# qcraftai/gedepth

Hardware: AMD Instinct MI355X
Metric: training img/s (whole node), KITTI-shaped 352x1120 synthetic batches (higher is better)
Workload: dtype bf16; 1 GPU; depthformer_swint_v: DepthFormer-SwinT + GEDepth-Vanilla, 352x1120, 8 img/GPU, full train step; global_batch=8, parallelism=dp1, allreduce_dtype=fp32, layout=nhwc, window_attention=bf16 mfma, params=53516992, hip_graph=off

## Files before the change

gedepth_amd/csrc/msda.h:

```cpp
#pragma once
#include <limits.h>
#include "common.h"

#define MSDA_MAX_L 8
struct MsdaLevels { int H[MSDA_MAX_L]; int W[MSDA_MAX_L]; int start[MSDA_MAX_L]; };

template <typename T> struct Lanes;
template <> struct Lanes<float> { static constexpr int CPL = 4; };
template <> struct Lanes<bf16_t> { static constexpr int CPL = 8; };

#define MSDA_XCDS 8
__device__ __forceinline__ long msda_xcd_block(unsigned bid, unsigned nblk) {
  return (long)(bid % MSDA_XCDS) * (nblk / MSDA_XCDS) + bid / MSDA_XCDS;
}
static inline unsigned msda_grid(long n_items, int per_block) {
  return (ge_blocks(n_items, per_block, INT_MAX - MSDA_XCDS) + MSDA_XCDS - 1) / MSDA_XCDS * MSDA_XCDS;
}

typedef ge_u32x4 lw_raw_t;
template <typename T> struct RowDot;
template <> struct RowDot<float> {
  static __device__ __forceinline__ float dot(const lw_raw_t& a, const lw_raw_t& b) {
    float s = 0.f;
#pragma unroll
    for (int i = 0; i < 4; ++i) s += __uint_as_float(a[i]) * __uint_as_float(b[i]);
    return s;
  }
};
template <> struct RowDot<bf16_t> {
  static __device__ __forceinline__ float dot(const lw_raw_t& a, const lw_raw_t& b) {
    const unsigned int a0 = a.x, a1 = a.y, a2 = a.z, a3 = a.w, b0 = b.x, b1 = b.y, b2 = b.z, b3 = b.w;
    float s = 0.f;
    s = __builtin_amdgcn_fdot2_f32_bf16(__builtin_bit_cast(ge_bf16x2, a0), __builtin_bit_cast(ge_bf16x2, b0), s, false);
    s = __builtin_amdgcn_fdot2_f32_bf16(__builtin_bit_cast(ge_bf16x2, a1), __builtin_bit_cast(ge_bf16x2, b1), s, false);
    s = __builtin_amdgcn_fdot2_f32_bf16(__builtin_bit_cast(ge_bf16x2, a2), __builtin_bit_cast(ge_bf16x2, b2), s, false);
    s = __builtin_amdgcn_fdot2_f32_bf16(__builtin_bit_cast(ge_bf16x2, a3), __builtin_bit_cast(ge_bf16x2, b3), s, false);
    return s;
  }
};

__device__ __forceinline__ int mul24(int a, int b) { return __mul24(a, b); }

static inline int msda_levels(const int* spatial_hw, int L, int Nv, MsdaLevels& lv) {
  if (L < 1 || L > MSDA_MAX_L) return GE_ERR_UNSUPPORTED;
  long start = 0;
  for (int l = 0; l < L; ++l) {
    lv.H[l] = spatial_hw[2 * l]; lv.W[l] = spatial_hw[2 * l + 1]; lv.start[l] = (int)start;
    if (lv.H[l] <= 0 || lv.W[l] <= 0) return GE_ERR_BAD_ARG;
    if ((long)lv.H[l] * lv.W[l] >= (1L << 23)) return GE_ERR_UNSUPPORTED;
    start += (long)lv.H[l] * lv.W[l];
  }
  return start == Nv ? GE_OK : GE_ERR_BAD_ARG;
}

#define MSDA_TW 8
#define MSDA_TH 4
#define MSDA_TILE 32
#define MSDA_CHUNK 4096
typedef float f32x32_t __attribute__((ext_vector_type(32)));
typedef float f32x2_t __attribute__((ext_vector_type(2)));
struct MsdaBins { int first_tile[MSDA_MAX_L + 1]; int ntx[MSDA_MAX_L]; };

struct MsdaWs {
  int* cnt; int* seg_hist; int* chunk_first; long* offset; int* ctrl; int4* entries;
  int* order;
};

int msda_drain_mfma_launch(const MsdaLevels& lv, const MsdaBins& bins, const MsdaWs& ws, const void* gout, float* d_value, int nbins,
                           int Nv, int Nq, int nH, int L, bool tr, hipStream_t s, bool rec8 = false);

int msda_win_supported(int B, int Nq, int nH, int L, int P, int Nv);
int msda_fwd_win_launch(const void* value, const MsdaLevels& lv, const int* query_hw, int n_qseg, const float* loc, const float* attw,
                        void* out, int B, int Nv, int Nq, int nH, int L, int P, int dtype, bool pre, hipStream_t s);
struct MwRaw {
  const void* off; long off_ld; const void* logit; long logit_ld;
  const float* ref; long ref_sb, ref_sq, ref_sl;
  float* loc_out; float* attw_out;
};
int msda_fwd_win_raw_launch(const void* value, const MsdaLevels& lv, const int* query_hw, int n_qseg, const MwRaw& rw, void* out, int B,
                            int Nv, int Nq, int nH, int L, int P, int dtype, hipStream_t s);
int msda_bwd_lw_win_launch(const void* value, const MsdaLevels& lv, const int* query_hw, int n_qseg, const float* loc,
                           const float* attw, const void* gout, float* d_loc, float* d_attw, int B, int Nv, int Nq, int nH, int L,
                           int P, int dtype, bool pre, hipStream_t s);
```

gedepth_amd/csrc/msda.hip:

```cpp
#include <algorithm>
#include <cstdlib>
#include "common.h"
#include "msda.h"
#include <string.h>
#include <mutex>
#include <vector>

__device__ __forceinline__ long msda_group(long v, int Nq, int nH, bool hm) {
  if (!hm) return v;
  const long bh = v / Nq;
  const long q = v - bh * Nq;
  const long b = bh / nH;
  return (b * Nq + q) * nH + (bh - b * nH);
}

template <typename T, bool HM>
__global__ void __launch_bounds__(256) msda_fwd_k(const T* __restrict__ value, MsdaLevels lv, const float* __restrict__ loc,
                                                  const float* __restrict__ attw, T* __restrict__ out,
                                                  long n_groups, int Nv, int Nq, int nH, int L, int P) {
  constexpr int CPL = Lanes<T>::CPL, G = 64 / CPL;
  const int c0 = (threadIdx.x % G) * CPL;
  const int nh64 = nH * 64;
  const long grp0 = msda_xcd_block(blockIdx.x, gridDim.x) * (blockDim.x / G) + (threadIdx.x / G);
  const long gstride = (long)gridDim.x * (blockDim.x / G);
// ... 495 lines not shown
            const float lg = bf2f(lgr[t]);
            const float e = __expf(lg - msda_half_max(lg));
            wgt = e * (1.f / msda_half_sum(e));
          }
          slot[s][0] = slot[s][1] = slot[s][2] = slot[s][3] = -1;
          key[s] = 0; packed[s] = 0;
          if (live && level_on && y > -1.f && x > -1.f && y < fH && x < fW) {
            const float xf = floorf(x), yf = floorf(y);
            const int x0 = (int)xf, y0 = (int)yf;
            const float ax = x - xf, ay = y - yf;
            const bool xa = x0 >= 0, xb = x0 + 1 < Wl, ya = y0 >= 0, yb = y0 + 1 < Hl;
            const int txa = x0 >> 3, txb = (x0 + 1) >> 3, tya = y0 >> 2, tyb = (y0 + 1) >> 2;
            const int tx = xa ? txa : txb, ty = ya ? tya : tyb;
            const bool two_x = xa && xb && txb != txa, two_y = ya && yb && tyb != tya;
            int* h0 = hist + lb0 + mul24(ty, ntx) + tx;
            const int lx1 = x0 - tx * MSDA_TW + 1, ly1 = y0 - ty * MSDA_TH + 1;
            key[s] = ((q_lo + (j >> 5)) << 7) | (ly1 << 4) | lx1;
            packed[s] = (uint32_t)f2bf(wgt) | ((uint32_t)min((int)(ax * 256.f), 255) << 16) | ((uint32_t)min((int)(ay * 256.f), 255) << 24);
            slot[s][0] = atomicAdd(h0, 1);
            if (two_x) slot[s][1] = atomicAdd(h0 + 1, 1);
            if (two_y) {
              slot[s][2] = atomicAdd(h0 + ntx, 1);
              if (two_x) slot[s][3] = atomicAdd(h0 + ntx + 1, 1);
            }
          }
        }
        if (FILL) {
          int2* rec = (int2*)ws.entries;
#pragma unroll
          for (int s = 0; s < S; ++s) {
            if (slot[s][0] >= 0) rec[slot[s][0]] = make_int2(key[s], (int)packed[s]);
            if (slot[s][1] >= 0) rec[slot[s][1]] = make_int2(key[s] & ~15, (int)packed[s]);
            if (slot[s][2] >= 0) rec[slot[s][2]] = make_int2(key[s] & ~0x70, (int)packed[s]);
            if (slot[s][3] >= 0) rec[slot[s][3]] = make_int2(key[s] & ~0x7f, (int)packed[s]);
          }
        }
      }
    }
    __syncthreads();
    if (!FILL) {
      for (int i = threadIdx.x; i < ntiles; i += 1024) {
        const int c = hist[i];
        gh[i] = c;
        if (c) atomicAdd(&ws.cnt[bh * ntiles + i], c);
      }
      __syncthreads();
    }
  }
}

__global__ void __launch_bounds__(256) msda_segscan_k(MsdaWs ws, int ntiles, int R, int nbins) {
  const int i = blockIdx.x * blockDim.x + threadIdx.x;
  if (i >= nbins) return;
  const int bh = i / ntiles, tile = i - bh * ntiles;
  int run = (int)ws.offset[i];
  int* p = ws.seg_hist + (long)bh * R * ntiles + tile;
  for (int r = 0; r < R; ++r) { const int c = p[(long)r * ntiles]; p[(long)r * ntiles] = run; run += c; }
}

__device__ __forceinline__ void msda_wave_scan(long& vo, int& vk, int lane) {
#pragma unroll
  for (int d = 1; d < 64; d <<= 1) {
    const long o = __shfl_up(vo, d, 64);
    const int k = __shfl_up(vk, d, 64);
    if (lane >= d) { vo += o; vk += k; }
  }
}
__global__ void __launch_bounds__(1024) msda_scan_k(MsdaWs ws, int nbins) {
  __shared__ long w_off[16];
  __shared__ int w_chk[16];
  const int lane = threadIdx.x & 63, wv = threadIdx.x >> 6;
  const int seg = ((nbins + 15) / 16 + 511) / 512 * 512;
  const int lo = wv * seg, hi = min(nbins, lo + seg);
  auto load8 = [&](int i0, int* c) {
    if (i0 + 8 <= hi) {
      const int4 a = *(const int4*)(ws.cnt + i0), b = *(const int4*)(ws.cnt + i0 + 4);
      c[0] = a.x; c[1] = a.y; c[2] = a.z; c[3] = a.w; c[4] = b.x; c[5] = b.y; c[6] = b.z; c[7] = b.w;
    } else {
#pragma unroll
      for (int e = 0; e < 8; ++e) c[e] = i0 + e < hi ? ws.cnt[i0 + e] : 0;
    }
  };
  long to = 0; int tk = 0;
  for (int base = lo; base < hi; base += 512) {
    int c[8];
    load8(base + lane * 8, c);
#pragma unroll
    for (int e = 0; e < 8; ++e) { to += c[e]; tk += (c[e] + MSDA_CHUNK - 1) / MSDA_CHUNK; }
  }
#pragma unroll
  for (int d = 32; d; d >>= 1) { to += __shfl_xor(to, d, 64); tk += __shfl_xor(tk, d, 64); }
  if (lane == 0) { w_off[wv] = to; w_chk[wv] = tk; }
  __syncthreads();
  long run_o = 0; int run_k = 0;
  for (int w = 0; w < wv; ++w) { run_o += w_off[w]; run_k += w_chk[w]; }
  for (int base = lo; base < hi; base += 512) {
    const int i0 = base + lane * 8;
    int c[8], kc[8];
    load8(i0, c);
    long vo = 0; int vk = 0;
#pragma unroll
    for (int e = 0; e < 8; ++e) { kc[e] = (c[e] + MSDA_CHUNK - 1) / MSDA_CHUNK; vo += c[e]; vk += kc[e]; }
    long so = vo; int sk = vk;
    msda_wave_scan(so, sk, lane);
    long o = run_o + so - vo; int k = run_k + sk - vk;
#pragma unroll
// ... 33 lines not shown
      int r = 0;
      for (int c = 0; c < nch; ++c) {
        const long slot = off0 + (long)c * MSDA_CHUNK;
        while (r + 1 < R && seg[(long)(r + 1) * ntiles + tile] <= slot) ++r;
        const int k = atomicAdd(&s_cnt[r], 1);
        if (pass) ws.order[first + s_base[r] + k] = c0 + c;
      }
    }
    __syncthreads();
    if (pass == 0) {
      if (threadIdx.x == 0) { int run = 0; for (int i = 0; i < R; ++i) { s_base[i] = run; run += s_cnt[i]; s_cnt[i] = 0; } }
      __syncthreads();
    }
  }
}

#define MSDA_SUB 512
#define MSDA_NCLS 45
template <typename T>
__global__ void __launch_bounds__(256) msda_drain_k(MsdaLevels lv, MsdaBins bins, MsdaWs ws, const T* __restrict__ gout,
                                                    float* __restrict__ d_value, int nbins, int Nv, int Nq, int nH, int L) {
  constexpr int CPLr = 16 / (int)sizeof(T);
  constexpr int LPR = 64 / CPLr;
  constexpr int RPI = 64 / LPR;
  constexpr int NR = 32 / RPI;
  __shared__ __attribute__((aligned(16))) T stage_all[4 * 32 * 64];
  __shared__ int s_key_all[4 * MSDA_SUB];
  __shared__ float s_w_all[4 * MSDA_SUB], s_ax_all[4 * MSDA_SUB], s_ay_all[4 * MSDA_SUB];
  __shared__ int s_start_all[4 * 64];
  const int lane = threadIdx.x & 63, wv = threadIdx.x >> 6;
  T* stage = stage_all + (size_t)wv * (32 * 64);
  int* s_key = s_key_all + wv * MSDA_SUB;
  float* s_w = s_w_all + wv * MSDA_SUB;
  float* s_ax = s_ax_all + wv * MSDA_SUB;
  float* s_ay = s_ay_all + wv * MSDA_SUB;
  int* s_start = s_start_all + wv * 64;
  const int gi = lane / LPR, subc = (lane % LPR) * CPLr;
  const int ntiles = bins.first_tile[L];
  const int total = ws.ctrl[0];
  const int part0 = blockIdx.x % MSDA_XCDS;
  int probe = 0;
  for (;;) {
    int item = -1;
    while (probe < MSDA_XCDS) {
      const int part = (part0 + probe) % MSDA_XCDS;
      const int p_lo = (int)((long)total * part / MSDA_XCDS), p_hi = (int)((long)total * (part + 1) / MSDA_XCDS);
      int k = 0;
      if (lane == 0) k = atomicAdd(&ws.ctrl[2 + part], 1);
      k = __builtin_amdgcn_readfirstlane(k);
      if (p_lo + k < p_hi) { item = p_lo + k; break; }
      ++probe;
    }
    if (item < 0) break;
    if (ws.order) item = ws.order[item];
    int lo = 0, hi = nbins;
    while (hi - lo > 1) { const int mid = (lo + hi) >> 1; if (ws.chunk_first[mid] <= item) lo = mid; else hi = mid; }
    const int bin = lo;
    const int nchunk = ws.chunk_first[bin + 1] - ws.chunk_first[bin];
    const int chunk = item - ws.chunk_first[bin];
    const int cnt = ws.cnt[bin];
    const int e_lo = chunk * MSDA_CHUNK, e_hi = min(cnt, e_lo + MSDA_CHUNK);
    const int4* ent = ws.entries + ws.offset[bin];
    const int bh = bin / ntiles, tile = bin - bh * ntiles;
    const int b = bh / nH, head = bh - b * nH;
    int l = 0;
    while (l + 1 < L && tile >= bins.first_tile[l + 1]) ++l;
    const int tl = tile - bins.first_tile[l];
    const int ty = tl / bins.ntx[l], tx = tl - ty * bins.ntx[l];
    const long rowbase = (long)b * Nq * nH + head;

    f32x32_t a0 = 0.f;
    for (int s_lo = e_lo; s_lo < e_hi; s_lo += MSDA_SUB) {
      const int n = min(MSDA_SUB, e_hi - s_lo);
      __builtin_amdgcn_wave_barrier();
      s_start[lane] = 0;
      __builtin_amdgcn_wave_barrier();
      int4 E[MSDA_SUB / 64];
      int rank[MSDA_SUB / 64];
#pragma unroll
      for (int i = 0; i < MSDA_SUB / 64; ++i) {
        const int idx = i * 64 + lane;
        E[i] = make_int4(0, 0, 0, 0);
        rank[i] = 0;
        if (idx < n) {
          E[i] = ent[s_lo + idx];
          rank[i] = atomicAdd(&s_start[((E[i].x >> 4) & 7) * 9 + (E[i].x & 15)], 1);
        }
      }
      __builtin_amdgcn_wave_barrier();
      {
        const int c = lane < MSDA_NCLS ? s_start[lane] : 0;
        int inc = c;
#pragma unroll
        for (int d = 1; d < 64; d <<= 1) { const int t = __shfl_up(inc, d, 64); if (lane >= d) inc += t; }
        __builtin_amdgcn_wave_barrier();
        s_start[lane] = lane < MSDA_NCLS ? inc - c : (lane == MSDA_NCLS ? n : 0x7fffffff);
      }
      __builtin_amdgcn_wave_barrier();
#pragma unroll
      for (int i = 0; i < MSDA_SUB / 64; ++i) {
        const int idx = i * 64 + lane;
        if (idx < n) {
          const int slot = s_start[((E[i].x >> 4) & 7) * 9 + (E[i].x & 15)] + rank[i];
          s_key[slot] = E[i].x;
          s_w[slot] = __int_as_float(E[i].y);
          s_ax[slot] = __int_as_float(E[i].z);
          s_ay[slot] = __int_as_float(E[i].w);
        }
      }
      const int nb = (n + 31) >> 5;
// ... 45 lines not shown
              accT = f32x2_t{carry ? accT.y : 0.f, 0.f};
              accB = f32x2_t{carry ? accB.y : 0.f, 0.f};
              ++cls;
              run_end = __builtin_amdgcn_readfirstlane(s_start[min(cls + 1, MSDA_NCLS + 1)]);
              rel = run_end - i0;
            } while (k == rel);
          }
          const f32x2_t kT = {nTx, nTy}, kB = {nBx, nBy};
          if (k + 1 < 32) {
            nTx = readlane_f(cT.x, k + 1); nTy = readlane_f(cT.y, k + 1); nBx = readlane_f(cB.x, k + 1); nBy = readlane_f(cB.y, k + 1);
          }
          const float g = gr[k];
          const f32x2_t g2 = {g, g};
          accT += kT * g2;
          accB += kB * g2;
        }
        if (blk + 1 < nb) { MSDA_PARK() }
      }
      {
        const int ly = cls / 9 - 1, lx = cls % 9 - 1;
        const bool in_cls = cls < MSDA_NCLS;
        MSDA_PUT(ly * MSDA_TW + lx, in_cls && ly >= 0 && lx >= 0, accT.x);
        MSDA_PUT((ly + 1) * MSDA_TW + lx, in_cls && ly < MSDA_TH - 1 && lx >= 0, accB.x);
        MSDA_PUT(ly * MSDA_TW + lx + 1, in_cls && ly >= 0 && lx < MSDA_TW - 1, accT.y);
        MSDA_PUT((ly + 1) * MSDA_TW + lx + 1, in_cls && ly < MSDA_TH - 1 && lx < MSDA_TW - 1, accB.y);
      }
#undef MSDA_GATHER
#undef MSDA_PARK
#undef MSDA_PUT
    }
    const int Wl = lv.W[l], Hl = lv.H[l];
    float* dst = d_value + (((long)b * Nv + lv.start[l]) * nH + head) * 64 + lane;
    const long pstride = (long)nH * 64;
#pragma unroll
    for (int e = 0; e < 32; ++e) {
      const int y = ty * MSDA_TH + e / MSDA_TW, x = tx * MSDA_TW + e % MSDA_TW;
      if (y < Hl && x < Wl) {
        float* p = dst + ((long)y * Wl + x) * pstride;
        if (nchunk == 1) *p = a0[e];
        else atomicAdd(p, a0[e]);
      }
    }
  }
}

static size_t msda_ws_layout(int nbins, long seg_hist_ints, long max_entries, char* base, MsdaWs* ws) {
  size_t off = 0;
  auto carve = [&](size_t bytes) { size_t o = off; off += (bytes + 255) / 256 * 256; return o; };
  const size_t o_cnt = carve((size_t)nbins * 4), o_chk = carve((size_t)(nbins + 1) * 4);
  const size_t o_off = carve((size_t)(nbins + 1) * 8), o_ctrl = carve(64), o_sh = carve((size_t)seg_hist_ints * 4);
  const size_t o_ord = carve((size_t)(nbins + max_entries / MSDA_CHUNK + 1) * 4);
  const size_t o_ent = carve((size_t)max_entries * 16);
  if (ws) {
    ws->order = (int*)(base + o_ord);
    ws->cnt = (int*)(base + o_cnt); ws->chunk_first = (int*)(base + o_chk); ws->offset = (long*)(base + o_off);
    ws->ctrl = (int*)(base + o_ctrl); ws->seg_hist = (int*)(base + o_sh); ws->entries = (int4*)(base + o_ent);
  }
  return off;
}
struct MsdaPlan { int ntiles, nloc, R, nbins; long max_entries; bool ok; };
#ifndef MSDA_HIST_WGS
#define MSDA_HIST_WGS 512
#endif
static MsdaPlan msda_plan(const MsdaBins& bins, int B, int Nq, int nH, int L, int P) {
  MsdaPlan pl;
  pl.ntiles = bins.first_tile[L];
  pl.nloc = nH * pl.ntiles;
  const long npts_b = (long)Nq * nH * L * P;
  long R = (MSDA_HIST_WGS + (long)B * nH - 1) / std::max(1L, (long)B * nH);
  R = std::max(1L, std::min(R, (long)std::max(1, Nq / 64)));
  pl.R = (int)R;
  pl.max_entries = (long)B * npts_b * 4;
  const long nbins = (long)B * pl.nloc;
  pl.nbins = (int)nbins;
  const size_t hist_bytes = (size_t)pl.ntiles * 4;
  pl.ok = nbins < (1L << 30) && Nq < (1 << 24) && pl.max_entries < (1L << 31) && hist_bytes <= 60 * 1024 && B <= 65535 &&
          ((long)Nq / R + 1) * L * P < (1L << 31) && (long)B * nH * R * pl.ntiles < (1L << 31) && R <= MSDA_MAX_R;
  return pl;
}
static int msda_bins(const MsdaLevels& lv, int L, MsdaBins& bins) {
  int n = 0;
  for (int l = 0; l < L; ++l) {
    bins.first_tile[l] = n;
    bins.ntx[l] = (lv.W[l] + MSDA_TW - 1) / MSDA_TW;
    n += bins.ntx[l] * ((lv.H[l] + MSDA_TH - 1) / MSDA_TH);
  }
  bins.first_tile[L] = n;
  return n;
}

static int g_msda_mode = 13 | 16 | 32;
extern "C" int ge_msda_mode(int mode) {
  const int old = g_msda_mode;
  if (mode >= 0) g_msda_mode = mode & 127;
  return old;
}

extern "C" int ge_msda_fwd(const void* value, const int* spatial_hw, const int* query_hw, int n_qseg, const float* loc,
                           const float* attw, void* out, int B, int Nv, int Nq, int nH, int L, int P, int dtype, void* stream) {
  if (!value || !spatial_hw || !loc || !attw || !out || B < 0 || Nv <= 0 || Nq < 0 || nH <= 0 || P <= 0) return GE_ERR_BAD_ARG;
  MsdaLevels lv;
  int e = msda_levels(spatial_hw, L, Nv, lv);
  if (e) return e;
  const long n_groups = (long)B * Nq * nH;
  if (n_groups == 0) return GE_OK;
  if (dtype != GE_F32 && dtype != GE_BF16) return GE_ERR_UNSUPPORTED;
  if ((g_msda_mode & 1) && query_hw && n_qseg > 0 && msda_win_supported(B, Nq, nH, L, P, Nv))
    return msda_fwd_win_launch(value, lv, query_hw, n_qseg, loc, attw, out, B, Nv, Nq, nH, L, P, dtype, (g_msda_mode & 4) != 0, ge_stream(stream));
  if ((n_groups + 15) / 16 > (1L << 30) || (long)Nv * nH * 64 >= (1L << 31)) return GE_ERR_UNSUPPORTED;
  const unsigned blocks = msda_grid(n_groups, dtype == GE_BF16 ? 32 : 16);
  const bool hm = (g_msda_mode & 8) != 0;
// ... 105 lines not shown
  const long seg_ints = (long)B * nH * pl.R * pl.ntiles;
  const bool binned = workspace && pl.ok && workspace_bytes >= msda_ws_layout(pl.nbins, seg_ints, pl.max_entries, nullptr, nullptr);
  if (!binned) {
    if (em || value_only) return GE_ERR_UNSUPPORTED;
    if (dtype == GE_F32) MSDA_BWD_P(float, true); else MSDA_BWD_P(bf16_t, true);
    GE_LAUNCH_CHECK();
    return GE_OK;
  }
#undef MSDA_BWD_P
#undef MSDA_BWD
  hipEvent_t evs[MSDA_NSTAGE + 1];
  hipEvent_t* ev = nullptr;
  { std::lock_guard<std::mutex> lk(g_msda_mu); if (g_msda_timing) ev = evs; }
  msda_mark(ev, 0, s);
  if (value_only) {
  } else if (em) {
    if (L != 4 || P != 8) return GE_ERR_UNSUPPORTED;
    const unsigned lblocks = msda_grid(n_groups, dtype == GE_BF16 ? 32 : 16);
    const bool hm = (g_msda_mode & 8) != 0;
    g_msda_lw_win_used = false;
#define MSDA_LWE(TT, HM_) msda_bwd_lw_k<TT, HM_, true><<<lblocks, 256, 0, s>>>((const TT*)value, lv, loc, attw, (const TT*)d_out, nullptr, nullptr, n_groups, Nv, Nq, nH, L, P, *em)
    if (dtype == GE_F32) { if (hm) MSDA_LWE(float, true); else MSDA_LWE(float, false); }
    else { if (hm) MSDA_LWE(bf16_t, true); else MSDA_LWE(bf16_t, false); }
#undef MSDA_LWE
  } else if ((g_msda_mode & 2) && query_hw && n_qseg > 0 && msda_win_supported(B, Nq, nH, L, P, Nv)) {
    e = msda_bwd_lw_win_launch(value, lv, query_hw, n_qseg, loc, attw, d_out, d_loc, d_attw, B, Nv, Nq, nH, L, P, dtype, (g_msda_mode & 4) != 0, s);
    if (e) return e;
    g_msda_lw_win_used = true;
  } else {
    const unsigned lblocks = msda_grid(n_groups, dtype == GE_BF16 ? 32 : 16);
    const bool hm = (g_msda_mode & 8) != 0;
    g_msda_lw_win_used = false;
#define MSDA_LW(TT, HM_) msda_bwd_lw_k<TT, HM_><<<lblocks, 256, 0, s>>>((const TT*)value, lv, loc, attw, (const TT*)d_out, d_loc, d_attw, n_groups, Nv, Nq, nH, L, P)
    if (dtype == GE_F32) { if (hm) MSDA_LW(float, true); else MSDA_LW(float, false); }
    else { if (hm) MSDA_LW(bf16_t, true); else MSDA_LW(bf16_t, false); }
#undef MSDA_LW
  }
  GE_LAUNCH_CHECK();
  msda_mark(ev, 1, s);
  if (!d_value) {
    if (ev) { std::lock_guard<std::mutex> lk(g_msda_mu); g_msda_pending.push_back(MsdaStageRec{0, ev[0], ev[1]}); }
    return GE_OK;
  }
  const int nbins = pl.nbins;
  MsdaWs ws;
  msda_ws_layout(nbins, seg_ints, pl.max_entries, (char*)workspace, &ws);
  hipError_t he = hipMemsetAsync(ws.cnt, 0, (size_t)nbins * 4, s);
  if (he != hipSuccess) return (int)he;
  const unsigned hgrid = (unsigned)std::min((long)MSDA_HIST_WGS, (long)B * nH * pl.R);
  const size_t hsmem = (size_t)pl.ntiles * 4;
  msda_hist_k<false><<<hgrid, 1024, hsmem, s>>>(lv, bins, loc, attw, ws, Nq, nH, L, P, pl.R, B);
  GE_LAUNCH_CHECK();
  msda_mark(ev, 2, s);
  msda_scan_k<<<1, 1024, 0, s>>>(ws, nbins);
  GE_LAUNCH_CHECK();
  msda_segscan_k<<<(unsigned)((nbins + 255) / 256), 256, 0, s>>>(ws, pl.ntiles, pl.R, nbins);
  GE_LAUNCH_CHECK();
  if (g_msda_mode & 64) {
    msda_order_k<<<(unsigned)(B * nH), 1024, 0, s>>>(ws, pl.ntiles, pl.R, 1);
    GE_LAUNCH_CHECK();
  } else ws.order = nullptr;
  msda_mark(ev, 3, s);
  msda_hist_k<true><<<hgrid, 1024, hsmem, s>>>(lv, bins, loc, attw, ws, Nq, nH, L, P, pl.R, B);
  GE_LAUNCH_CHECK();
  msda_mark(ev, 4, s);
  g_msda_drain_mfma_used = dtype == GE_BF16 && (g_msda_mode & 16);
  if (dtype == GE_F32)
    msda_drain_k<float><<<256 * 3, 256, 0, s>>>(lv, bins, ws, (const float*)d_out, d_value, nbins, Nv, Nq, nH, L);
  else if (g_msda_drain_mfma_used) {
    e = msda_drain_mfma_launch(lv, bins, ws, d_out, d_value, nbins, Nv, Nq, nH, L, (g_msda_mode & 32) != 0, s);
    if (e) return e;
  } else
    msda_drain_k<bf16_t><<<256 * 3, 256, 0, s>>>(lv, bins, ws, (const bf16_t*)d_out, d_value, nbins, Nv, Nq, nH, L);
  GE_LAUNCH_CHECK();
  msda_mark(ev, 5, s);
  if (ev) {
    std::lock_guard<std::mutex> lk(g_msda_mu);
    for (int i = 0; i < MSDA_NSTAGE; ++i) g_msda_pending.push_back(MsdaStageRec{i, ev[i], ev[i + 1]});
  }
  return GE_OK;
}

extern "C" int ge_msda_bwd(const void* value, const int* spatial_hw, const int* query_hw, int n_qseg, const float* loc,
                           const float* attw, const void* d_out, float* d_value, float* d_loc, float* d_attw, void* workspace,
                           size_t workspace_bytes, int B, int Nv, int Nq, int nH, int L, int P, int dtype, void* stream) {
  return msda_bwd_impl(value, spatial_hw, query_hw, n_qseg, loc, attw, d_out, d_value, d_loc, d_attw, workspace, workspace_bytes, B, Nv, Nq,
                       nH, L, P, dtype, stream, nullptr);
}

extern "C" int ge_msda_bwd_value(const void* value, const int* spatial_hw, const float* loc, const float* attw, const void* d_out,
                                 float* d_value, void* workspace, size_t workspace_bytes, int B, int Nv, int Nq, int nH, int L, int P,
                                 int dtype, void* stream) {
  return msda_bwd_impl(value, spatial_hw, nullptr, 0, loc, attw, d_out, d_value, nullptr, nullptr, workspace, workspace_bytes, B, Nv, Nq,
                       nH, L, P, dtype, stream, nullptr, true);
}

extern "C" int ge_msda_bwd_value_raw(const int* spatial_hw, const void* off_raw, long off_ld, const void* logit_raw, long logit_ld,
                                     const float* ref, long ref_sb, long ref_sq, long ref_sl, const void* d_out, float* d_value,
                                     void* workspace, size_t workspace_bytes, int B, int Nv, int Nq, int nH, int L, int P, int dtype,
                                     void* stream) {
  return ge_msda_bwd_value_raw_levels(spatial_hw, off_raw, off_ld, logit_raw, logit_ld, ref, ref_sb, ref_sq, ref_sl, d_out, d_value, workspace,
                                      workspace_bytes, 15, B, Nv, Nq, nH, L, P, dtype, stream);
}

extern "C" int ge_msda_bwd_value_raw_levels(const int* spatial_hw, const void* off_raw, long off_ld, const void* logit_raw, long logit_ld,
                                            const float* ref, long ref_sb, long ref_sq, long ref_sl, const void* d_out, float* d_value,
                                            void* workspace, size_t workspace_bytes, int level_mask, int B, int Nv, int Nq, int nH, int L,
                                            int P, int dtype, void* stream) {
  if (!spatial_hw || !off_raw || !logit_raw || !ref || !d_out || !d_value || !workspace || B < 0 || Nq < 0 || nH <= 0) return GE_ERR_BAD_ARG;
  if (dtype != GE_BF16 || L != 4 || P != 8) return GE_ERR_UNSUPPORTED;
  MsdaLevels lv;
  int e = msda_levels(spatial_hw, L, Nv, lv);
  if (e) return e;
  for (int l = 0; l < L; ++l) if (lv.W[l] > 8191 || lv.H[l] > 8191) return GE_ERR_UNSUPPORTED;
  if ((long)B * Nq * nH == 0) return GE_OK;
  MsdaBins bins;
  msda_bins(lv, L, bins);
  const MsdaPlan pl = msda_plan(bins, B, Nq, nH, L, P);
  const long seg_ints = (long)B * nH * pl.R * pl.ntiles;
  if (!pl.ok || workspace_bytes < msda_ws_layout(pl.nbins, seg_ints, pl.max_entries, nullptr, nullptr)) return GE_ERR_UNSUPPORTED;
  hipStream_t s = ge_stream(stream);
  MsdaRawIn in;
  in.off = (const bf16_t*)off_raw; in.off_ld = off_ld; in.logit = (const bf16_t*)logit_raw; in.logit_ld = logit_ld;
  in.ref = ref; in.ref_sb = ref_sb; in.ref_sq = ref_sq; in.ref_sl = ref_sl;
  for (int l = 0; l < 4; ++l) { in.fW[l] = (float)lv.W[l]; in.fH[l] = (float)lv.H[l]; in.rW[l] = 1.f / in.fW[l]; in.rH[l] = 1.f / in.fH[l]; }
  hipEvent_t evs[MSDA_NSTAGE + 1];
  hipEvent_t* ev = nullptr;
  { std::lock_guard<std::mutex> lk(g_msda_mu); if (g_msda_timing) ev = evs; }
  msda_mark(ev, 0, s);
  msda_mark(ev, 1, s);
  const int nbins = pl.nbins;
  MsdaWs ws;
  msda_ws_layout(nbins, seg_ints, pl.max_entries, (char*)workspace, &ws);
  hipError_t he = hipMemsetAsync(ws.cnt, 0, (size_t)nbins * 4, s);
  if (he != hipSuccess) return (int)he;
  const unsigned hgrid = (unsigned)std::min((long)MSDA_HIST_WGS, (long)B * nH * pl.R);
  const size_t hsmem = (size_t)pl.ntiles * 4;
  msda_hist_raw_k<false, MSDA_HIST_UC, 1><<<hgrid, 1024, hsmem, s>>>(lv, bins, in, ws, Nq, nH, pl.R, B, level_mask);
  GE_LAUNCH_CHECK();
  msda_mark(ev, 2, s);
  msda_scan_k<<<1, 1024, 0, s>>>(ws, nbins);
  GE_LAUNCH_CHECK();
  msda_segscan_k<<<(unsigned)((nbins + 255) / 256), 256, 0, s>>>(ws, pl.ntiles, pl.R, nbins);
  GE_LAUNCH_CHECK();
  if (g_msda_mode & 64) {
    msda_order_k<<<(unsigned)(B * nH), 1024, 0, s>>>(ws, pl.ntiles, pl.R, 1);
    GE_LAUNCH_CHECK();
  } else ws.order = nullptr;
  msda_mark(ev, 3, s);
  msda_hist_raw_k<true, MSDA_HIST_UF, MSDA_HIST_S><<<hgrid, 1024, hsmem, s>>>(lv, bins, in, ws, Nq, nH, pl.R, B, level_mask);
  GE_LAUNCH_CHECK();
  msda_mark(ev, 4, s);
  g_msda_drain_mfma_used = true;
  g_msda_lw_win_used = false;
  e = msda_drain_mfma_launch(lv, bins, ws, d_out, d_value, nbins, Nv, Nq, nH, L, true, s, true);
  if (e) return e;
  msda_mark(ev, 5, s);
  if (ev) {
    std::lock_guard<std::mutex> lk(g_msda_mu);
    for (int i = 0; i < MSDA_NSTAGE; ++i) g_msda_pending.push_back(MsdaStageRec{i, ev[i], ev[i + 1]});
  }
  return GE_OK;
}

template <typename T, int K>
__device__ __forceinline__ void ld_run(const T* p, float* v) {
  constexpr int VN = V8<T>::N;
  if constexpr (K % VN == 0) {
#pragma unroll
    for (int i = 0; i < K; i += VN) V8<T>::ld(p + i, v + i);
  } else {
#pragma unroll
    for (int i = 0; i < K; ++i) v[i] = Io<T>::ld(p + i);
  }
}
template <typename T, int K>
__device__ __forceinline__ void st_run(T* p, const float* v) {
  constexpr int VN = V8<T>::N;
  if constexpr (K % VN == 0) {
#pragma unroll
    for (int i = 0; i < K; i += VN) V8<T>::st(p + i, v + i);
  } else {
#pragma unroll
    for (int i = 0; i < K; ++i) Io<T>::st(p + i, v[i]);
  }
}

template <typename T, int P>
__global__ void __launch_bounds__(256) msda_prep_fwd_k(const T* __restrict__ off_raw, long off_ld, const T* __restrict__ logit_raw,
                                                       long logit_ld, const float* __restrict__ ref, long ref_sb, long ref_sq,
                                                       long ref_sl, MsdaLevels lv, float* __restrict__ loc, float* __restrict__ attw,
                                                       long total, int Nq, int nH) {
  for (long t = (long)blockIdx.x * 256 + threadIdx.x; t < total; t += (long)gridDim.x * 256) {
    const int l = (int)(t & 3);
    const long g = t >> 2;
    const int h = (int)(g % nH);
    const long row = g / nH;
    const long b = row / Nq, q = row - b * Nq;
    float off[2 * P], lg[P];
    ld_run<T, 2 * P>(off_raw + row * off_ld + ((long)h * 4 + l) * (2 * P), off);
    ld_run<T, P>(logit_raw + row * logit_ld + ((long)h * 4 + l) * P, lg);
// ... 205 lines not shown
```

gedepth_amd/csrc/msda_drain_mfma.hip:

```cpp
#include "msda.h"

#define MD_BLK 64
#define MD_HALF (MD_BLK * 32 + 32)
#define MD_STAGE (2 * MD_HALF)
#define MD_AIMG (MD_BLK * 32)

template <bool REC8> struct MdRec;
typedef int md_i32x4 __attribute__((ext_vector_type(4)));
typedef int md_i32x2 __attribute__((ext_vector_type(2)));
template <> struct MdRec<false> {
  typedef int4 T;
  static __device__ __forceinline__ T load(const T* p) { const md_i32x4 v = __builtin_nontemporal_load((const md_i32x4*)p); return make_int4(v.x, v.y, v.z, v.w); }
  static __device__ __forceinline__ T pad(int key) { return make_int4(key, 0, 0, 0); }
  static __device__ __forceinline__ int key(const T& e) { return e.x; }
  static __device__ __forceinline__ void coef(const T& e, float& w, float& ax, float& ay) { w = __int_as_float(e.y); ax = __int_as_float(e.z); ay = __int_as_float(e.w); }
};
template <> struct MdRec<true> {
  typedef int2 T;
  static __device__ __forceinline__ T load(const T* p) { const md_i32x2 v = __builtin_nontemporal_load((const md_i32x2*)p); return make_int2(v.x, v.y); }
  static __device__ __forceinline__ T pad(int key) { return make_int2(key, 0); }
  static __device__ __forceinline__ int key(const T& e) { return e.x; }
  static __device__ __forceinline__ void coef(const T& e, float& w, float& ax, float& ay) {
    w = __uint_as_float((uint32_t)e.y << 16);
    ax = ((float)(((uint32_t)e.y >> 16) & 255u) + 0.5f) * (1.f / 256.f);
    ay = ((float)((uint32_t)e.y >> 24) + 0.5f) * (1.f / 256.f);
  }
};

template <bool TR, bool REC8>
__global__ void __launch_bounds__(256) msda_drain_mfma_k(MsdaLevels lv, MsdaBins bins, MsdaWs ws, const bf16_t* __restrict__ gout,
                                                         float* __restrict__ d_value, int nbins, int Nv, int Nq, int nH, int L) {
  __shared__ __attribute__((aligned(16))) bf16_t stage_all[4 * MD_STAGE];
  __shared__ __attribute__((aligned(16))) bf16_t aimg_all[4 * MD_AIMG];
  const int lane = threadIdx.x & 63, wv = threadIdx.x >> 6;
  bf16_t* stage = stage_all + wv * MD_STAGE;
  bf16_t* aimg = aimg_all + wv * MD_AIMG;
  {
    const uint4 z = make_uint4(0, 0, 0, 0);
#pragma unroll
    for (int i = 0; i < MD_AIMG / (64 * 8); ++i) *(uint4*)(aimg + (i * 64 + lane) * 8) = z;
  }
  const int ntiles = bins.first_tile[L];
  const int total = ws.ctrl[0];
  const int part0 = blockIdx.x % MSDA_XCDS;
  const int sub8 = lane & 7, row8 = lane >> 3;
  const int park_off = (sub8 >> 2) * MD_HALF + (sub8 & 3) * 8;
  const int a_rec = ((lane >> 4) * 2 + ((lane >> 3) & 1)) * 256 + (lane & 7);
  const int tr_row = (lane >> 5) * 8 + ((lane & 15) >> 2), tr_col = ((lane >> 4) & 1) * 16 + (lane & 3) * 4;
  int probe = 0;
  for (;;) {
    int item = -1;
    while (probe < MSDA_XCDS) {
      const int part = (part0 + probe) % MSDA_XCDS;
      const int p_lo = (int)((long)total * part / MSDA_XCDS), p_hi = (int)((long)total * (part + 1) / MSDA_XCDS);
      int k = 0;
      if (lane == 0) k = atomicAdd(&ws.ctrl[2 + part], 1);
      k = __builtin_amdgcn_readfirstlane(k);
      if (p_lo + k < p_hi) { item = p_lo + k; break; }
      ++probe;
    }
    if (item < 0) break;
    if (ws.order) item = ws.order[item];
    int lo = 0, hi = nbins;
    while (hi - lo > 1) { const int mid = (lo + hi) >> 1; if (ws.chunk_first[mid] <= item) lo = mid; else hi = mid; }
    const int bin = lo;
    const int nchunk = ws.chunk_first[bin + 1] - ws.chunk_first[bin];
    const int chunk = item - ws.chunk_first[bin];
    const int cnt = ws.cnt[bin];
    const int e_lo = chunk * MSDA_CHUNK, e_hi = min(cnt, e_lo + MSDA_CHUNK);
    typedef typename MdRec<REC8>::T rec_t;
    const rec_t* ent = (const rec_t*)ws.entries + ws.offset[bin] + e_lo;
    const int n = e_hi - e_lo;
    const int bh = bin / ntiles, tile = bin - bh * ntiles;
    const int b = bh / nH, head = bh - b * nH;
    int l = 0;
    while (l + 1 < L && tile >= bins.first_tile[l + 1]) ++l;
    const int tl = tile - bins.first_tile[l];
    const int ty = tl / bins.ntx[l], tx = tl - ty * bins.ntx[l];
    const bf16_t* grow = gout + ((long)b * Nq * nH + head) * 64 + sub8 * 8;
    const int qpitch = nH * 64;

    ge_f32x16 acc0 = 0.f, acc1 = 0.f;
    const int nb = (n + MD_BLK - 1) / MD_BLK;
    ge_u32x4 R[8];
    rec_t E0, E1, E2;
    const rec_t padrec = MdRec<REC8>::pad(MdRec<REC8>::key(ent[0]));
#define MD_LOAD(DST, BLK) { DST = padrec; if ((BLK) * MD_BLK + lane < n) DST = MdRec<REC8>::load(ent + (BLK) * MD_BLK + lane); }
#define MD_GATHER(EE)                                                                          \
  _Pragma("unroll") for (int i = 0; i < 8; ++i) {                                              \
    const int q = __shfl(MdRec<REC8>::key(EE) >> 7, i * 8 + row8, 64);                                       \
    R[i] = *(const ge_u32x4*)(grow + (long)q * qpitch);                                         \
  }
#define MD_PARK()                                                                              \
  _Pragma("unroll") for (int i = 0; i < 8; ++i) *(ge_u32x4*)(stage + park_off + (i * 8 + row8) * 32) = R[i];
#define MD_COEF(EE, ZERO)                                                                      \
  {                                                                                            \
    const int lx = (MdRec<REC8>::key(EE) & 15) - 1, ly = ((MdRec<REC8>::key(EE) >> 4) & 7) - 1; \
    float w, ax, ay;                                                                            \
    MdRec<REC8>::coef(EE, w, ax, ay);                                                           \
    const bool xl = lx >= 0, xr = lx < MSDA_TW - 1, yt = ly >= 0, yb = ly < MSDA_TH - 1;        \
    const float wl = 1.f - ax, wt = w * (1.f - ay), wb = w * ay;                                \
    bf16_t* a00 = aimg + a_rec + (ly * MSDA_TW + lx) * 8;                                       \
    if (yt && xl) a00[0] = (ZERO) ? (bf16_t)0 : f2bf_hw(wt * wl);                                 \
    if (yt && xr) a00[8] = (ZERO) ? (bf16_t)0 : f2bf_hw(wt * ax);                                 \
    if (yb && xl) a00[MSDA_TW * 8] = (ZERO) ? (bf16_t)0 : f2bf_hw(wb * wl);                       \
    if (yb && xr) a00[MSDA_TW * 8 + 8] = (ZERO) ? (bf16_t)0 : f2bf_hw(wb * ax);                   \
  }
    MD_LOAD(E0, 0)
    MD_LOAD(E1, 1)
    MD_GATHER(E0)
    __builtin_amdgcn_wave_barrier();
    MD_COEF(E0, false)
    MD_PARK()
    __builtin_amdgcn_wave_barrier();
    for (int blk = 0; blk < nb; ++blk) {
      const bool more = blk + 1 < nb;
      if (more) { MD_GATHER(E1) }
      MD_LOAD(E2, blk + 2)
#pragma unroll
      for (int ks = 0; ks < 4; ++ks) {
        const ge_bf16x8 A = *(const ge_bf16x8*)(aimg + ((ks * 2 + (lane >> 5)) * 32 + (lane & 31)) * 8);
#pragma unroll
        for (int half = 0; half < 2; ++half) {
          ge_bf16x8 Bv;
          if (TR) {
            const bf16_t* p = stage + half * MD_HALF + (ks * 16 + tr_row) * 32 + tr_col;
            const ge_bf16x4 t0 = __builtin_amdgcn_ds_read_tr16_b64_v4bf16(GE_LDS(ge_bf16x4, p));
            const ge_bf16x4 t1 = __builtin_amdgcn_ds_read_tr16_b64_v4bf16(GE_LDS(ge_bf16x4, p + 4 * 32));
            Bv = __builtin_shufflevector(t0, t1, 0, 1, 2, 3, 4, 5, 6, 7);
          } else {
            const bf16_t* p = stage + half * MD_HALF + (ks * 16 + (lane >> 5) * 8) * 32 + (lane & 31);
            uint32_t wq[4];
#pragma unroll
            for (int e = 0; e < 4; ++e) wq[e] = (uint32_t)p[(2 * e) * 32] | ((uint32_t)p[(2 * e + 1) * 32] << 16);
            Bv = __builtin_bit_cast(ge_bf16x8, make_uint4(wq[0], wq[1], wq[2], wq[3]));
          }
          if (half == 0) acc0 = __builtin_amdgcn_mfma_f32_32x32x16_bf16(A, Bv, acc0, 0, 0, 0);
          else acc1 = __builtin_amdgcn_mfma_f32_32x32x16_bf16(A, Bv, acc1, 0, 0, 0);
        }
      }
      __builtin_amdgcn_wave_barrier();
      MD_COEF(E0, true)
      if (more) {
        MD_COEF(E1, false)
        MD_PARK()
      }
      __builtin_amdgcn_wave_barrier();
      E0 = E1; E1 = E2;
    }
#undef MD_LOAD
#undef MD_GATHER
#undef MD_PARK
#undef MD_COEF
    const int Wl = lv.W[l], Hl = lv.H[l];
    float* dst = d_value + (((long)b * Nv + lv.start[l]) * nH + head) * 64 + (lane & 31);
    const long pstride = (long)nH * 64;
#pragma unroll
    for (int r = 0; r < 16; ++r) {
      const int m = (r & 3) + 8 * (r >> 2) + 4 * (lane >> 5);
      const int y = ty * MSDA_TH + m / MSDA_TW, x = tx * MSDA_TW + m % MSDA_TW;
      if (y < Hl && x < Wl) {
        float* p = dst + ((long)y * Wl + x) * pstride;
        if (nchunk == 1) { p[0] = acc0[r]; p[32] = acc1[r]; }
        else { atomicAdd(p, acc0[r]); atomicAdd(p + 32, acc1[r]); }
      }
    }
  }
}

int msda_drain_mfma_launch(const MsdaLevels& lv, const MsdaBins& bins, const MsdaWs& ws, const void* gout, float* d_value, int nbins,
                           int Nv, int Nq, int nH, int L, bool tr, hipStream_t s, bool rec8) {
  if (rec8) msda_drain_mfma_k<true, true><<<256 * 3, 256, 0, s>>>(lv, bins, ws, (const bf16_t*)gout, d_value, nbins, Nv, Nq, nH, L);
  else if (tr) msda_drain_mfma_k<true, false><<<256 * 3, 256, 0, s>>>(lv, bins, ws, (const bf16_t*)gout, d_value, nbins, Nv, Nq, nH, L);
  else msda_drain_mfma_k<false, false><<<256 * 3, 256, 0, s>>>(lv, bins, ws, (const bf16_t*)gout, d_value, nbins, Nv, Nq, nH, L);
  GE_LAUNCH_CHECK();
  return GE_OK;
}
```

Measured before the change: 172.1 img/s.

## Deepen MSDA drain gather ring and precompute chunk-to-bin map

The MFMA drain kernel for the deformable-attention backward value gradient now keeps a ring of D gathered blocks and 2D entry records in flight, unrolling the block loop so that global gathers run further ahead of the MFMA work. It also sets an occupancy hint of three waves per SIMD, makes scalar values wave-uniform with readfirstlane, and clears coefficients by the previous key rather than through a separate zero pass. When ordering is off, the segscan kernel fills a chunk-to-bin table so the drain can skip its per-item binary search. The deeper ring raises register pressure, which the static_assert notes could spill.

```diff
diff --git a/gedepth_amd/csrc/msda.h b/gedepth_amd/csrc/msda.h
--- a/gedepth_amd/csrc/msda.h
+++ b/gedepth_amd/csrc/msda.h
@@ -56,7 +56,9 @@
 #define MSDA_TW 8
 #define MSDA_TH 4
 #define MSDA_TILE 32
+#ifndef MSDA_CHUNK
 #define MSDA_CHUNK 4096
+#endif
 typedef float f32x32_t __attribute__((ext_vector_type(32)));
 typedef float f32x2_t __attribute__((ext_vector_type(2)));
 struct MsdaBins { int first_tile[MSDA_MAX_L + 1]; int ntx[MSDA_MAX_L]; };
@@ -64,7 +66,16 @@
 struct MsdaWs {
   int* cnt; int* seg_hist; int* chunk_first; long* offset; int* ctrl; int4* entries;
   int* order;
+  int* chunk_bin;
 };
+
+__device__ __forceinline__ int msda_chunk_bin(const MsdaWs& ws, int& item, int nbins) {
+  if (ws.chunk_bin) return ws.chunk_bin[item];
+  item = ws.order[item];
+  int lo = 0, hi = nbins;
+  while (hi - lo > 1) { const int mid = (lo + hi) >> 1; if (ws.chunk_first[mid] <= item) lo = mid; else hi = mid; }
+  return lo;
+}
 
 int msda_drain_mfma_launch(const MsdaLevels& lv, const MsdaBins& bins, const MsdaWs& ws, const void* gout, float* d_value, int nbins,
                            int Nv, int Nq, int nH, int L, bool tr, hipStream_t s, bool rec8 = false);
diff --git a/gedepth_amd/csrc/msda.hip b/gedepth_amd/csrc/msda.hip
--- a/gedepth_amd/csrc/msda.hip
+++ b/gedepth_amd/csrc/msda.hip
@@ -571,6 +571,7 @@
 __global__ void __launch_bounds__(256) msda_segscan_k(MsdaWs ws, int ntiles, int R, int nbins) {
   const int i = blockIdx.x * blockDim.x + threadIdx.x;
   if (i >= nbins) return;
+  if (ws.chunk_bin) for (int ch = ws.chunk_first[i], end = ws.chunk_first[i + 1]; ch < end; ++ch) ws.chunk_bin[ch] = i;
   const int bh = i / ntiles, tile = i - bh * ntiles;
   int run = (int)ws.offset[i];
   int* p = ws.seg_hist + (long)bh * R * ntiles + tile;
@@ -710,10 +711,7 @@
       ++probe;
     }
     if (item < 0) break;
-    if (ws.order) item = ws.order[item];
-    int lo = 0, hi = nbins;
-    while (hi - lo > 1) { const int mid = (lo + hi) >> 1; if (ws.chunk_first[mid] <= item) lo = mid; else hi = mid; }
-    const int bin = lo;
+    const int bin = msda_chunk_bin(ws, item, nbins);
     const int nchunk = ws.chunk_first[bin + 1] - ws.chunk_first[bin];
     const int chunk = item - ws.chunk_first[bin];
     const int cnt = ws.cnt[bin];
@@ -865,11 +863,14 @@
   const size_t o_ord = carve((size_t)(nbins + max_entries / MSDA_CHUNK + 1) * 4);
   const size_t o_ent = carve((size_t)max_entries * 16);
   if (ws) {
-    ws->order = (int*)(base + o_ord);
+    ws->order = (int*)(base + o_ord); ws->chunk_bin = nullptr;
     ws->cnt = (int*)(base + o_cnt); ws->chunk_first = (int*)(base + o_chk); ws->offset = (long*)(base + o_off);
     ws->ctrl = (int*)(base + o_ctrl); ws->seg_hist = (int*)(base + o_sh); ws->entries = (int4*)(base + o_ent);
   }
   return off;
+}
+static void msda_ws_order(MsdaWs& ws, bool grouped) {
+  if (!grouped) { ws.chunk_bin = ws.order; ws.order = nullptr; }
 }
 struct MsdaPlan { int ntiles, nloc, R, nbins; long max_entries; bool ok; };
 #ifndef MSDA_HIST_WGS
@@ -1081,6 +1082,7 @@
   msda_hist_k<false><<<hgrid, 1024, hsmem, s>>>(lv, bins, loc, attw, ws, Nq, nH, L, P, pl.R, B);
   GE_LAUNCH_CHECK();
   msda_mark(ev, 2, s);
+  msda_ws_order(ws, (g_msda_mode & 64) != 0);
   msda_scan_k<<<1, 1024, 0, s>>>(ws, nbins);
   GE_LAUNCH_CHECK();
   msda_segscan_k<<<(unsigned)((nbins + 255) / 256), 256, 0, s>>>(ws, pl.ntiles, pl.R, nbins);
@@ -1088,7 +1090,7 @@
   if (g_msda_mode & 64) {
     msda_order_k<<<(unsigned)(B * nH), 1024, 0, s>>>(ws, pl.ntiles, pl.R, 1);
     GE_LAUNCH_CHECK();
-  } else ws.order = nullptr;
+  }
   msda_mark(ev, 3, s);
   msda_hist_k<true><<<hgrid, 1024, hsmem, s>>>(lv, bins, loc, attw, ws, Nq, nH, L, P, pl.R, B);
   GE_LAUNCH_CHECK();
@@ -1168,6 +1170,7 @@
   msda_hist_raw_k<false, MSDA_HIST_UC, 1><<<hgrid, 1024, hsmem, s>>>(lv, bins, in, ws, Nq, nH, pl.R, B, level_mask);
   GE_LAUNCH_CHECK();
   msda_mark(ev, 2, s);
+  msda_ws_order(ws, (g_msda_mode & 64) != 0);
   msda_scan_k<<<1, 1024, 0, s>>>(ws, nbins);
   GE_LAUNCH_CHECK();
   msda_segscan_k<<<(unsigned)((nbins + 255) / 256), 256, 0, s>>>(ws, pl.ntiles, pl.R, nbins);
@@ -1175,7 +1178,7 @@
   if (g_msda_mode & 64) {
     msda_order_k<<<(unsigned)(B * nH), 1024, 0, s>>>(ws, pl.ntiles, pl.R, 1);
     GE_LAUNCH_CHECK();
-  } else ws.order = nullptr;
+  }
   msda_mark(ev, 3, s);
   msda_hist_raw_k<true, MSDA_HIST_UF, MSDA_HIST_S><<<hgrid, 1024, hsmem, s>>>(lv, bins, in, ws, Nq, nH, pl.R, B, level_mask);
   GE_LAUNCH_CHECK();
diff --git a/gedepth_amd/csrc/msda_drain_mfma.hip b/gedepth_amd/csrc/msda_drain_mfma.hip
--- a/gedepth_amd/csrc/msda_drain_mfma.hip
+++ b/gedepth_amd/csrc/msda_drain_mfma.hip
@@ -27,9 +27,21 @@
   }
 };
 
+#ifndef MD_RING
+#define MD_RING 2
+#endif
+static_assert(MD_RING >= 1 && MD_RING <= 2, "gather ring depth: 3 sets spill at three waves per SIMD");
+
+__device__ __forceinline__ int md_uni(int v) { return __builtin_amdgcn_readfirstlane(v); }
+__device__ __forceinline__ long md_uni(long v) { return (long)(((unsigned long)(unsigned)md_uni((int)(v >> 32)) << 32) | (unsigned)md_uni((int)v)); }
+
+struct MdFlush { float* dst; int Wl, Hl, ty, tx; bool single; };
+
 template <bool TR, bool REC8>
-__global__ void __launch_bounds__(256) msda_drain_mfma_k(MsdaLevels lv, MsdaBins bins, MsdaWs ws, const bf16_t* __restrict__ gout,
+__global__ void __launch_bounds__(256, 3) msda_drain_mfma_k(MsdaLevels lv, MsdaBins bins, MsdaWs ws, const bf16_t* __restrict__ gout,
                                                          float* __restrict__ d_value, int nbins, int Nv, int Nq, int nH, int L) {
+  constexpr int D = MD_RING, NE = 2 * D;
+  typedef typename MdRec<REC8>::T rec_t;
   __shared__ __attribute__((aligned(16))) bf16_t stage_all[4 * MD_STAGE];
   __shared__ __attribute__((aligned(16))) bf16_t aimg_all[4 * MD_AIMG];
   const int lane = threadIdx.x & 63, wv = threadIdx.x >> 6;
@@ -47,125 +59,158 @@
   const int park_off = (sub8 >> 2) * MD_HALF + (sub8 & 3) * 8;
   const int a_rec = ((lane >> 4) * 2 + ((lane >> 3) & 1)) * 256 + (lane & 7);
   const int tr_row = (lane >> 5) * 8 + ((lane & 15) >> 2), tr_col = ((lane >> 4) & 1) * 16 + (lane & 3) * 4;
+  const int qpitch = nH * 64;
+
   int probe = 0;
-  for (;;) {
-    int item = -1;
+  auto next_item = [&]() -> int {
     while (probe < MSDA_XCDS) {
       const int part = (part0 + probe) % MSDA_XCDS;
       const int p_lo = (int)((long)total * part / MSDA_XCDS), p_hi = (int)((long)total * (part + 1) / MSDA_XCDS);
       int k = 0;
       if (lane == 0) k = atomicAdd(&ws.ctrl[2 + part], 1);
-      k = __builtin_amdgcn_readfirstlane(k);
-      if (p_lo + k < p_hi) { item = p_lo + k; break; }
+      k = md_uni(k);
+      if (p_lo + k < p_hi) return p_lo + k;
       ++probe;
     }
-    if (item < 0) break;
-    if (ws.order) item = ws.order[item];
-    int lo = 0, hi = nbins;
-    while (hi - lo > 1) { const int mid = (lo + hi) >> 1; if (ws.chunk_first[mid] <= item) lo = mid; else hi = mid; }
-    const int bin = lo;
-    const int nchunk = ws.chunk_first[bin + 1] - ws.chunk_first[bin];
-    const int chunk = item - ws.chunk_first[bin];
-    const int cnt = ws.cnt[bin];
-    const int e_lo = chunk * MSDA_CHUNK, e_hi = min(cnt, e_lo + MSDA_CHUNK);
-    typedef typename MdRec<REC8>::T rec_t;
-    const rec_t* ent = (const rec_t*)ws.entries + ws.offset[bin] + e_lo;
-    const int n = e_hi - e_lo;
+    return -1;
+  };
+
+  const rec_t* ent = nullptr;
+  const bf16_t* grow = nullptr;
+  int n = 0, nb = 0;
+  rec_t padrec = MdRec<REC8>::pad(0);
+  MdFlush fl = {nullptr, 0, 0, 0, 0, true};
+  rec_t E[NE];
+#define MD_LOAD(DST, BLK) DST = MdRec<REC8>::load(ent + min((BLK) * MD_BLK + lane, n - 1));
+#define MD_PAD(DST, BLK) if ((BLK) * MD_BLK + lane >= n) DST = padrec;
+  auto open_chunk = [&](int item, int bin, int cnt, long off, int cf0, int cf1) {
+    bin = md_uni(bin); cnt = md_uni(cnt); off = md_uni(off); cf0 = md_uni(cf0); cf1 = md_uni(cf1);
+    const int e_lo = (item - cf0) * MSDA_CHUNK;
+    n = min(cnt, e_lo + MSDA_CHUNK) - e_lo;
+    nb = (n + MD_BLK - 1) / MD_BLK;
+    ent = (const rec_t*)ws.entries + off + e_lo;
     const int bh = bin / ntiles, tile = bin - bh * ntiles;
     const int b = bh / nH, head = bh - b * nH;
     int l = 0;
     while (l + 1 < L && tile >= bins.first_tile[l + 1]) ++l;
     const int tl = tile - bins.first_tile[l];
-    const int ty = tl / bins.ntx[l], tx = tl - ty * bins.ntx[l];
-    const bf16_t* grow = gout + ((long)b * Nq * nH + head) * 64 + sub8 * 8;
-    const int qpitch = nH * 64;
-
+    fl.ty = tl / bins.ntx[l]; fl.tx = tl - fl.ty * bins.ntx[l];
+    fl.Wl = lv.W[l]; fl.Hl = lv.H[l];
+    fl.single = cf1 - cf0 == 1;
+    fl.dst = d_value + (((long)b * Nv + lv.start[l]) * nH + head) * 64;
+    grow = gout + ((long)b * Nq * nH + head) * 64 + sub8 * 8;
+    padrec = MdRec<REC8>::pad(MdRec<REC8>::key(ent[0]));
+#pragma unroll
+    for (int j = 0; j < NE; ++j) MD_LOAD(E[j], j)
+  };
+  auto flush = [&](const MdFlush& f, const ge_f32x16& acc0, const ge_f32x16& acc1) {
+    float* dst = f.dst + (lane & 31);
+    const long pstride = (long)nH * 64;
+#pragma unroll
+    for (int r = 0; r < 16; ++r) {
+      const int m = (r & 3) + 8 * (r >> 2) + 4 * (lane >> 5);
+      const int y = f.ty * MSDA_TH + m / MSDA_TW, x = f.tx * MSDA_TW + m % MSDA_TW;
+      if (y < f.Hl && x < f.Wl) {
+        float* p = dst + ((long)y * f.Wl + x) * pstride;
+        if (f.single) { p[0] = acc0[r]; p[32] = acc1[r]; }
+        else { atomicAdd(p, acc0[r]); atomicAdd(p + 32, acc1[r]); }
+      }
+    }
+  };
+  auto a_put = [&](int key, bf16_t c00, bf16_t c01, bf16_t c10, bf16_t c11) {
+    const int lx = (key & 15) - 1, ly = ((key >> 4) & 7) - 1;
+    const bool xl = lx >= 0, xr = lx < MSDA_TW - 1, yt = ly >= 0, yb = ly < MSDA_TH - 1;
+    bf16_t* a00 = aimg + a_rec + (ly * MSDA_TW + lx) * 8;
+    if (yt && xl) a00[0] = c00;
+    if (yt && xr) a00[8] = c01;
+    if (yb && xl) a00[MSDA_TW * 8] = c10;
+    if (yb && xr) a00[MSDA_TW * 8 + 8] = c11;
+  };
+  auto a_write = [&](const rec_t& e) {
+    float w, ax, ay;
+    MdRec<REC8>::coef(e, w, ax, ay);
+    const float wl = 1.f - ax, wt = w * (1.f - ay), wb = w * ay;
+    a_put(MdRec<REC8>::key(e), f2bf_hw(wt * wl), f2bf_hw(wt * ax), f2bf_hw(wb * wl), f2bf_hw(wb * ax));
+  };
+
+  for (;;) {
+    int item = next_item();
+    if (item < 0) break;
+    {
+      const int bin = msda_chunk_bin(ws, item, nbins);
+      open_chunk(item, bin, ws.cnt[bin], ws.offset[bin], ws.chunk_first[bin], ws.chunk_first[bin + 1]);
+    }
     ge_f32x16 acc0 = 0.f, acc1 = 0.f;
-    const int nb = (n + MD_BLK - 1) / MD_BLK;
-    ge_u32x4 R[8];
-    rec_t E0, E1, E2;
-    const rec_t padrec = MdRec<REC8>::pad(MdRec<REC8>::key(ent[0]));
-#define MD_LOAD(DST, BLK) { DST = padrec; if ((BLK) * MD_BLK + lane < n) DST = MdRec<REC8>::load(ent + (BLK) * MD_BLK + lane); }
-#define MD_GATHER(EE)                                                                          \
+    ge_u32x4 R[D][8];
+#define MD_GATHER(RR, EE)                                                                      \
   _Pragma("unroll") for (int i = 0; i < 8; ++i) {                                              \
-    const int q = __shfl(MdRec<REC8>::key(EE) >> 7, i * 8 + row8, 64);                                       \
-    R[i] = *(const ge_u32x4*)(grow + (long)q * qpitch);                                         \
-  }
-#define MD_PARK()                                                                              \
-  _Pragma("unroll") for (int i = 0; i < 8; ++i) *(ge_u32x4*)(stage + park_off + (i * 8 + row8) * 32) = R[i];
-#define MD_COEF(EE, ZERO)                                                                      \
-  {                                                                                            \
-    const int lx = (MdRec<REC8>::key(EE) & 15) - 1, ly = ((MdRec<REC8>::key(EE) >> 4) & 7) - 1; \
-    float w, ax, ay;                                                                            \
-    MdRec<REC8>::coef(EE, w, ax, ay);                                                           \
-    const bool xl = lx >= 0, xr = lx < MSDA_TW - 1, yt = ly >= 0, yb = ly < MSDA_TH - 1;        \
-    const float wl = 1.f - ax, wt = w * (1.f - ay), wb = w * ay;                                \
-    bf16_t* a00 = aimg + a_rec + (ly * MSDA_TW + lx) * 8;                                       \
-    if (yt && xl) a00[0] = (ZERO) ? (bf16_t)0 : f2bf_hw(wt * wl);                                 \
-    if (yt && xr) a00[8] = (ZERO) ? (bf16_t)0 : f2bf_hw(wt * ax);                                 \
-    if (yb && xl) a00[MSDA_TW * 8] = (ZERO) ? (bf16_t)0 : f2bf_hw(wb * wl);                       \
-    if (yb && xr) a00[MSDA_TW * 8 + 8] = (ZERO) ? (bf16_t)0 : f2bf_hw(wb * ax);                   \
-  }
-    MD_LOAD(E0, 0)
-    MD_LOAD(E1, 1)
-    MD_GATHER(E0)
+    const int q = __shfl(MdRec<REC8>::key(EE) >> 7, i * 8 + row8, 64);                          \
+    RR[i] = *(const ge_u32x4*)(grow + (long)q * qpitch);                                        \
+  }
+#define MD_PARK(RR)                                                                            \
+  _Pragma("unroll") for (int i = 0; i < 8; ++i) *(ge_u32x4*)(stage + park_off + (i * 8 + row8) * 32) = RR[i];
+#pragma unroll
+    for (int j = 0; j < D; ++j) { MD_PAD(E[j], j) MD_GATHER(R[j], E[j]) }
     __builtin_amdgcn_wave_barrier();
-    MD_COEF(E0, false)
-    MD_PARK()
+    a_write(E[0]);
+    int zkey = MdRec<REC8>::key(E[0]);
+    MD_PARK(R[0])
     __builtin_amdgcn_wave_barrier();
-    for (int blk = 0; blk < nb; ++blk) {
-      const bool more = blk + 1 < nb;
-      if (more) { MD_GATHER(E1) }
-      MD_LOAD(E2, blk + 2)
-#pragma unroll
-      for (int ks = 0; ks < 4; ++ks) {
-        const ge_bf16x8 A = *(const ge_bf16x8*)(aimg + ((ks * 2 + (lane >> 5)) * 32 + (lane & 31)) * 8);
-#pragma unroll
-        for (int half = 0; half < 2; ++half) {
-          ge_bf16x8 Bv;
-          if (TR) {
-            const bf16_t* p = stage + half * MD_HALF + (ks * 16 + tr_row) * 32 + tr_col;
-            const ge_bf16x4 t0 = __builtin_amdgcn_ds_read_tr16_b64_v4bf16(GE_LDS(ge_bf16x4, p));
-            const ge_bf16x4 t1 = __builtin_amdgcn_ds_read_tr16_b64_v4bf16(GE_LDS(ge_bf16x4, p + 4 * 32));
-            Bv = __builtin_shufflevector(t0, t1, 0, 1, 2, 3, 4, 5, 6, 7);
-          } else {
-            const bf16_t* p = stage + half * MD_HALF + (ks * 16 + (lane >> 5) * 8) * 32 + (lane & 31);
-            uint32_t wq[4];
-#pragma unroll
-            for (int e = 0; e < 4; ++e) wq[e] = (uint32_t)p[(2 * e) * 32] | ((uint32_t)p[(2 * e + 1) * 32] << 16);
-            Bv = __builtin_bit_cast(ge_bf16x8, make_uint4(wq[0], wq[1], wq[2], wq[3]));
-          }
-          if (half == 0) acc0 = __builtin_amdgcn_mfma_f32_32x32x16_bf16(A, Bv, acc0, 0, 0, 0);
-          else acc1 = __builtin_amdgcn_mfma_f32_32x32x16_bf16(A, Bv, acc1, 0, 0, 0);
-        }
-      }
-      __builtin_amdgcn_wave_barrier();
-      MD_COEF(E0, true)
-      if (more) {
-        MD_COEF(E1, false)
-        MD_PARK()
-      }
-      __builtin_amdgcn_wave_barrier();
-      E0 = E1; E1 = E2;
-    }
-#undef MD_LOAD
+#define MD_BLOCK(u, blk, TAIL)                                                                                              \
+  {                                                                                                                 \
+    if (!(TAIL) || (blk) + D < nb) {                                                                                \
+      MD_PAD(E[(u + D) % NE], (blk) + D)                                                                            \
+      MD_GATHER(R[u % D], E[(u + D) % NE])                                                                          \
+    }                                                                                                               \
+    if (!(TAIL)) MD_LOAD(E[u], (blk) + NE)                                                                          \
+_Pragma("unroll")                                                                                                   \
+    for (int ks = 0; ks < 4; ++ks) {                                                                                \
+      const ge_bf16x8 A = *(const ge_bf16x8*)(aimg + ((ks * 2 + (lane >> 5)) * 32 + (lane & 31)) * 8);              \
+_Pragma("unroll")                                                                                                   \
+      for (int half = 0; half < 2; ++half) {                                                                        \
+        ge_bf16x8 Bv;                                                                                               \
+        if (TR) {                                                                                                   \
+          const bf16_t* p = stage + half * MD_HALF + (ks * 16 + tr_row) * 32 + tr_col;                              \
+          const ge_bf16x4 t0 = __builtin_amdgcn_ds_read_tr16_b64_v4bf16(GE_LDS(ge_bf16x4, p));                      \
+          const ge_bf16x4 t1 = __builtin_amdgcn_ds_read_tr16_b64_v4bf16(GE_LDS(ge_bf16x4, p + 4 * 32));             \
+          Bv = __builtin_shufflevector(t0, t1, 0, 1, 2, 3, 4, 5, 6, 7);                                             \
+        } else {                                                                                                    \
+          const bf16_t* p = stage + half * MD_HALF + (ks * 16 + (lane >> 5) * 8) * 32 + (lane & 31);                \
+          uint32_t wq[4];                                                                                           \
+_Pragma("unroll")                                                                                                   \
+          for (int e = 0; e < 4; ++e) wq[e] = (uint32_t)p[(2 * e) * 32] | ((uint32_t)p[(2 * e + 1) * 32] << 16);    \
+          Bv = __builtin_bit_cast(ge_bf16x8, make_uint4(wq[0], wq[1], wq[2], wq[3]));                               \
+        }                                                                                                           \
+        if (half == 0) acc0 = __builtin_amdgcn_mfma_f32_32x32x16_bf16(A, Bv, acc0, 0, 0, 0);                        \
+        else acc1 = __builtin_amdgcn_mfma_f32_32x32x16_bf16(A, Bv, acc1, 0, 0, 0);                                  \
+      }                                                                                                             \
+    }                                                                                                               \
+    __builtin_amdgcn_wave_barrier();                                                                                \
+    a_put(zkey, 0, 0, 0, 0);                                                                                        \
+    if (!(TAIL) || (blk) + 1 < nb) {                                                                                \
+      a_write(E[(u + 1) % NE]);                                                                                     \
+      zkey = MdRec<REC8>::key(E[(u + 1) % NE]);                                                                     \
+      MD_PARK(R[(u + 1) % D])                                                                                       \
+    }                                                                                                               \
+    __builtin_amdgcn_wave_barrier();                                                                                \
+  }
+    int blk0 = 0;
+    for (; blk0 + NE < nb; blk0 += NE) {
+#pragma unroll
+      for (int u = 0; u < NE; ++u) MD_BLOCK(u, blk0 + u, false)
+    }
+#pragma unroll
+    for (int u = 0; u < NE; ++u) {
+      if (blk0 + u >= nb) break;
+      MD_BLOCK(u, blk0 + u, true)
+    }
+#undef MD_BLOCK
 #undef MD_GATHER
 #undef MD_PARK
-#undef MD_COEF
-    const int Wl = lv.W[l], Hl = lv.H[l];
-    float* dst = d_value + (((long)b * Nv + lv.start[l]) * nH + head) * 64 + (lane & 31);
-    const long pstride = (long)nH * 64;
-#pragma unroll
-    for (int r = 0; r < 16; ++r) {
-      const int m = (r & 3) + 8 * (r >> 2) + 4 * (lane >> 5);
-      const int y = ty * MSDA_TH + m / MSDA_TW, x = tx * MSDA_TW + m % MSDA_TW;
-      if (y < Hl && x < Wl) {
-        float* p = dst + ((long)y * Wl + x) * pstride;
-        if (nchunk == 1) { p[0] = acc0[r]; p[32] = acc1[r]; }
-        else { atomicAdd(p, acc0[r]); atomicAdd(p + 32, acc1[r]); }
-      }
-    }
-  }
+    flush(fl, acc0, acc1);
+  }
+#undef MD_LOAD
+#undef MD_PAD
 }
 
 int msda_drain_mfma_launch(const MsdaLevels& lv, const MsdaBins& bins, const MsdaWs& ws, const void* gout, float* d_value, int nbins,
```

Measured after the change: 172.9 img/s, median of 3. About the same (+0.4%).
